# Atticuszz/GsplatLoc

Hardware: AMD Instinct MI355X
Metric: Gaussians/s fwd+bwd @1M splats 1200x680 (higher is better)
Workload: dtype f32

## Files before the change

### gsplatloc_amd/csrc/raster_g16.hip

```cpp
#include <stdlib.h>
#include <string.h>

#include "gsloc_common.h"

namespace gsl {

__device__ __forceinline__ float g16_sel(unsigned long long m, float t, float f) {
  float r;
  asm("v_cndmask_b32_e64 %0, %1, %2, %3" : "=v"(r) : "v"(f), "v"(t), "s"(m));
  return r;
}

#define G16_M_LO8 0x00FF00FF00FF00FFull
#define G16_M_B2 0x0F0F0F0F0F0F0F0Full
#define G16_M_B1 0x3333333333333333ull
#define G16_M_B0 0x5555555555555555ull

constexpr int G16_NG = GSL_NG;
constexpr int G16_GL = 64 / G16_NG;
static_assert(G16_NG == 4 || G16_NG == 8, "pixel groups are DPP rows or half rows");

__device__ __forceinline__ float row_scatter8(const float (&v)[8]) {
  float n0, n1, n2, n3, m0, m1;
  asm volatile(
      "s_nop 1\n\t"
      "v_add_f32_dpp %0, %6, %6 row_mirror row_mask:0xf bank_mask:0xf\n\t"
      "v_add_f32_dpp %1, %7, %7 row_mirror row_mask:0xf bank_mask:0xf\n\t"
      "v_add_f32_dpp %2, %8, %8 row_mirror row_mask:0xf bank_mask:0xf\n\t"
      "v_add_f32_dpp %3, %9, %9 row_mirror row_mask:0xf bank_mask:0xf\n\t"
      "v_add_f32_dpp %0, %10, %10 row_mirror row_mask:0xf bank_mask:0xc\n\t"
      "v_add_f32_dpp %1, %11, %11 row_mirror row_mask:0xf bank_mask:0xc\n\t"
      "v_add_f32_dpp %2, %12, %12 row_mirror row_mask:0xf bank_mask:0xc\n\t"
      "v_add_f32_dpp %4, %0, %0 row_half_mirror row_mask:0xf bank_mask:0xf\n\t"
      "v_add_f32_dpp %5, %1, %1 row_half_mirror row_mask:0xf bank_mask:0xf\n\t"
      "v_add_f32_dpp %4, %2, %2 row_half_mirror row_mask:0xf bank_mask:0xa\n\t"
      "v_add_f32_dpp %5, %3, %3 row_half_mirror row_mask:0xf bank_mask:0xa\n\t"
      : "=&v"(n0), "=&v"(n1), "=&v"(n2), "=&v"(n3), "=&v"(m0), "=&v"(m1)
      : "v"(v[0]), "v"(v[1]), "v"(v[2]), "v"(v[3]), "v"(v[4]), "v"(v[5]), "v"(v[6]));
  float keep = g16_sel(G16_M_B1, m0, m1), send = g16_sel(G16_M_B1, m1, m0);
  float r = keep + dpp_get<0x4E>(send);
  r += dpp_get<0xB1>(r);
  return r;
}

__device__ __forceinline__ float row_scatter16(const float (&v)[16]) {
  float a[8];
#pragma unroll
  for (int i = 0; i < 8; ++i) {
    float keep = g16_sel(G16_M_LO8, v[i], v[i + 8]), send = g16_sel(G16_M_LO8, v[i + 8], v[i]);
    a[i] = keep + dpp_get<0x140>(send);
  }
  float n[4], m[2];
#pragma unroll
  for (int i = 0; i < 4; ++i) {
    float keep = g16_sel(G16_M_B2, a[i], a[i + 4]), send = g16_sel(G16_M_B2, a[i + 4], a[i]);
    n[i] = keep + dpp_get<0x141>(send);
  }
#pragma unroll
  for (int i = 0; i < 2; ++i) {
    float keep = g16_sel(G16_M_B1, n[i], n[i + 2]), send = g16_sel(G16_M_B1, n[i + 2], n[i]);
    m[i] = keep + dpp_get<0x4E>(send);
  }
  float keep = g16_sel(G16_M_B0, m[0], m[1]), send = g16_sel(G16_M_B0, m[1], m[0]);
  return keep + dpp_get<0xB1>(send);
}

__device__ __forceinline__ float4 half_scatter8(const float (&v)[8]) {
  float n0, n1, n2, n3;
  asm volatile(
      "s_nop 1\n\t"
      "v_add_f32_dpp %0, %4, %4 row_half_mirror row_mask:0xf bank_mask:0xf\n\t"
      "v_add_f32_dpp %1, %5, %5 row_half_mirror row_mask:0xf bank_mask:0xf\n\t"
      "v_add_f32_dpp %2, %6, %6 row_half_mirror row_mask:0xf bank_mask:0xf\n\t"
      "v_add_f32_dpp %3, %7, %7 row_half_mirror row_mask:0xf bank_mask:0xf\n\t"
      "v_add_f32_dpp %0, %8, %8 row_half_mirror row_mask:0xf bank_mask:0xa\n\t"
      "v_add_f32_dpp %1, %9, %9 row_half_mirror row_mask:0xf bank_mask:0xa\n\t"
      "v_add_f32_dpp %2, %10, %10 row_half_mirror row_mask:0xf bank_mask:0xa\n\t"
      "s_nop 1\n\t"
      : "=&v"(n0), "=&v"(n1), "=&v"(n2), "=&v"(n3)
      : "v"(v[0]), "v"(v[1]), "v"(v[2]), "v"(v[3]), "v"(v[4]), "v"(v[5]), "v"(v[6]));
  n0 += dpp_get<0x4E>(n0); n1 += dpp_get<0x4E>(n1); n2 += dpp_get<0x4E>(n2); n3 += dpp_get<0x4E>(n3);
  n0 += dpp_get<0xB1>(n0); n1 += dpp_get<0xB1>(n1); n2 += dpp_get<0xB1>(n2); n3 += dpp_get<0xB1>(n3);
  return make_float4(n0, n1, n2, n3);
}

__device__ __forceinline__ void half_scatter16(const float (&v)[16], float4& lo, float4& hi) {
  float a[8];
#pragma unroll
  for (int i = 0; i < 8; ++i) {
    float keep = g16_sel(G16_M_B2, v[i], v[i + 8]), send = g16_sel(G16_M_B2, v[i + 8], v[i]);
    a[i] = keep + dpp_get<0x141>(send);
  }
#pragma unroll
  for (int i = 0; i < 8; ++i) a[i] += dpp_get<0x4E>(a[i]);
#pragma unroll
  for (int i = 0; i < 8; ++i) a[i] += dpp_get<0xB1>(a[i]);
  lo = make_float4(a[0], a[1], a[2], a[3]);
  hi = make_float4(a[4], a[5], a[6], a[7]);
}

#ifdef GSL_G16_STATS
__device__ unsigned long long g16_stats[8];
#define G16_STAT(i, n) do { unsigned long long n__ = (unsigned long long)(n); if (lane == 0) atomicAdd(&g16_stats[i], n__); } while (0)
#else
#define G16_STAT(i, n) do { } while (0)
#endif

#ifndef GSL_QB
#define GSL_QB 64
#endif
#define GSL_QBS (GSL_QB + 1)
#ifndef GSL_Q_LCAP
#define GSL_Q_LCAP 24
#endif

template <int D, int CG>
struct QStage {
  static constexpr int NV = 6 + CG;
  static constexpr int NS = (NV <= 8) ? 8 : 16;
  static constexpr int A = 6 + D;
  static constexpr int LCAP = ((NS == 8) ? GSL_Q_LCAP : GSL_Q_LCAP / 2) * 4 / G16_NG;
  float4 s0[GSL_QBS];
  float4 s1[GSL_QBS];
  float4 s2[(D >= 3 && CG == D) ? GSL_QBS : 1];
  int32_t id[GSL_QBS];
  uint32_t posn[G16_NG / 4][GSL_QBS];
  alignas(16) float pair[G16_NG * LCAP * NS];
  uint8_t rlist[G16_NG][GSL_QBS + 4];
  uint8_t nzlist[64];
};

template <int D, int CG>
__device__ __forceinline__ void qraster_bwd_body(
    QStage<D, CG>& sb, const float4* __restrict__ Q0, const float4* __restrict__ Q1, const float4* __restrict__ Q2,
    const uint4* __restrict__ Qh, const int32_t* __restrict__ flatten_ids, float* __restrict__ vacc, long long rs,
    long long re, int lane, int quad, float px, float py, float tx0, float ty0, int bin_final, float T_init,
    float Bp_init, const float (&vc)[D], const uint32_t* __restrict__ qhits, int n_qhits) {
  constexpr bool RGB = D >= 3;
  constexpr bool DEPTH = (D == 1) || (D == 4);
  constexpr int NV = QStage<D, CG>::NV;
  constexpr int NS = QStage<D, CG>::NS;
  constexpr int A = QStage<D, CG>::A;
  constexpr int LCAP = QStage<D, CG>::LCAP;
  constexpr int NG = G16_NG, GL = G16_GL;
  constexpr int PP = 12;
  static_assert(A <= PP && NG * LCAP * NS >= 64 * PP, "64 packed gradient rows reuse the pair slots");
  static_assert(GSL_QB < 127 && GSL_QB >= 64, "7-bit list positions with 127 reserved; a chunk appends up to 64 entries");
  const int grp = lane / GL, p = lane & (GL - 1);
  const float tcx = tx0 + 8.f, tcy = ty0 + 8.f;
  const float lx = px - tcx, ly = py - tcy;
  const float lxx = lx * lx, lxy = lx * ly, lyy = ly * ly;
  float T = T_init;
  float Bp = Bp_init;
  const int myslot = (NG == 8) ? (p >> 2) * (NS / 2) : ((NS == 8) ? (p >> 1) : p);
  const bool writer = (NG == 8) ? ((p & 3) == 0) : ((NS == 8) ? ((p & 1) == 0) : true);
  float* const mypair = &sb.pair[grp * LCAP * NS + myslot];
  uint8_t* const mylist = sb.rlist[grp];
  const unsigned long long lt = (1ull << lane) - 1ull;
  const float qx0 = tx0 + 8.f * (float)(quad & 1), qy0 = ty0 + 8.f * (float)(quad >> 1);
  int grp_final[NG];
  {
    int rf = bin_final;
    rf = max(rf, __shfl_xor(rf, 1, 64));
    rf = max(rf, __shfl_xor(rf, 2, 64));
    rf = max(rf, __shfl_xor(rf, 4, 64));
    if (GL == 16) rf = max(rf, __shfl_xor(rf, 8, 64));
#pragma unroll
    for (int g = 0; g < NG; ++g) grp_final[g] = __builtin_amdgcn_readlane(rf, GL * g);
  }
  if (lane == 0) {
    sb.s0[GSL_QB] = make_float4(0.f, 0.f, 0.f, 0.f);
    sb.s1[GSL_QB] = make_float4(0.f, 0.f, 0.f, 0.f);
    if (RGB && CG == D) sb.s2[GSL_QB] = make_float4(0.f, 0.f, 0.f, 0.f);
  }
  int pos = __builtin_amdgcn_readfirstlane(qhits ? n_qhits : (int)re);
  const int pos_end = __builtin_amdgcn_readfirstlane(qhits ? 0 : (int)rs);
  while (pos > pos_end) {
    int staged = 0;
    int cnt[NG];
#pragma unroll
    for (int g = 0; g < NG; ++g) cnt[g] = 0;
    __syncthreads();
    while (pos > pos_end && staged <= GSL_QB - 64) {
      long long idx = (long long)(pos - 1 - lane);
      bool in = idx >= (long long)pos_end;
      unsigned nib = 0;
      int gid = 0;
      float4 r0 = make_float4(0.f, 0.f, 0.f, 0.f), r1 = r0, r2 = r0;
      if (in) {
        if (qhits) {
          unsigned e = qhits[idx];
          nib = e >> GSL_HIT_SHIFT;
          idx = (long long)(e & GSL_HIT_INDEX_MASK);
          gid = flatten_ids[idx];
          load_record(Q0, Q1, Q2, Qh, gid, RGB && CG == D, r0, r1, r2);
        } else {
          gid = flatten_ids[idx];
          load_record(Q0, Q1, Q2, Qh, gid, RGB && CG == D, r0, r1, r2);
          if (r1.w >= 0.f) {
            float rr = r1.w * r1.w;
#pragma unroll
            for (int g = 0; g < NG; ++g) {
              const int b = (NG == 8) ? (g >> 1) : g;
              const float cy = (NG == 8) ? 2.f * (float)(g & 1) + 1.f : 2.f, hy = (NG == 8) ? 0.5f : 1.5f;
              float ex = fmaxf(fabsf(r0.x - (qx0 + 4.f * (float)(b & 1) + 2.f)) - 1.5f, 0.f);
              float ey = fmaxf(fabsf(r0.y - (qy0 + 4.f * (float)(b >> 1) + cy)) - hy, 0.f);
              bool h = (ex * ex + ey * ey <= rr) && ((int)idx <= grp_final[g]);
              nib |= (h ? 1u : 0u) << g;
            }
          }
        }
      }
      unsigned long long R = __ballot(nib != 0);
      int slot = staged + __popcll(R & lt);
      unsigned pack[NG / 4];
#pragma unroll
      for (int w = 0; w < NG / 4; ++w) pack[w] = 0x0FFFFFFFu;
#pragma unroll
      for (int g = 0; g < NG; ++g) {
        unsigned long long Bg = __ballot(nib & (1u << g));
        if (__builtin_amdgcn_inverse_ballot_w64(Bg)) {
          int q = cnt[g] + __popcll(Bg & lt);
          sb.rlist[g][q] = (uint8_t)slot;
          pack[g >> 2] ^= (127u ^ (unsigned)q) << (7 * (g & 3));
        }
        cnt[g] += __popcll(Bg);
      }
      if (__builtin_amdgcn_inverse_ballot_w64(R)) {
        sb.id[slot] = gid;
        sb.s0[slot] = r0;
        sb.s1[slot] = make_float4(r1.x * (0.5f * GSL_LOG2E), r1.y * GSL_LOG2E, r1.z * (0.5f * GSL_LOG2E),
                                  __int_as_float((int)idx));
        if (RGB && CG == D) sb.s2[slot] = r2;
#pragma unroll
        for (int w = 0; w < NG / 4; ++w) sb.posn[w][slot] = pack[w];
      }
      staged += __popcll(R);
      pos -= 64;
    }
    if (staged == 0) continue;
    int kmax = 0, cnt_tot = 0, cnt_my = 0;
#pragma unroll
    for (int g = 0; g < NG; ++g) {
      kmax = max(kmax, cnt[g]);
      cnt_tot += cnt[g];
      cnt_my = (grp == g) ? cnt[g] : cnt_my;
    }
    G16_STAT(6, kmax);
    G16_STAT(7, cnt_tot);
    (void)cnt_tot;
    for (int k = cnt_my + p; k < kmax + 3; k += GL) mylist[k] = (uint8_t)GSL_QB;
    __syncthreads();
    constexpr int NU = (GSL_QB + 63) / 64;
    float mo[NU][NV];
#pragma unroll
    for (int u = 0; u < NU; ++u)
#pragma unroll
      for (int q = 0; q < NV; ++q) mo[u][q] = 0.f;
    auto trip = [&](int t, const float4& c0, const float4& c1, float4& r, float4& r2) {
      float dx = c0.x - px, dy = c0.y - py;
      float sigma = fmaf(c1.y * dx, dy, fmaf(c1.x * dx, dx, c1.z * dy * dy));
      float vis = __builtin_amdgcn_exp2f(-sigma);
      float opv = c0.w * vis;
      float alpha = fminf(GSL_ALPHA_MAX, opv);
      unsigned long long validm = __ballot(__float_as_int(c1.w) <= bin_final) & __ballot(sigma >= 0.f) &
                                  __ballot(alpha >= GSL_ALPHA_MIN);
      G16_STAT(0, 1);
      r = make_float4(0.f, 0.f, 0.f, 0.f);
      r2 = r;
      if (validm) {
        G16_STAT(1, 1);
#ifdef GSL_G16_STATS
        {
          int groups_hit = 0;
          for (int g = 0; g < NG; ++g) groups_hit += ((validm >> (GL * g)) & ((1ull << GL) - 1ull)) != 0;
          G16_STAT(3, groups_hit);
        }
#endif
        G16_STAT(5, __popcll(validm));
        unsigned long long capm = __ballot(opv <= GSL_ALPHA_MAX);
        float am = g16_sel(validm, alpha, 0.f);
        float ra = __builtin_amdgcn_rcpf(1.f - am);
        T *= ra;
        float fac = am * T;
        float cdot;
        if (CG == D) {
          cdot = 0.f;
          if (RGB) {
            float4 q2 = sb.s2[t];
            cdot = q2.x * vc[0] + q2.y * vc[1] + q2.z * vc[2];
          }
          if (DEPTH) cdot += c0.z * vc[D - 1];
        } else {
          cdot = c0.z * vc[D - 1];
        }
        float v_alpha = T * cdot - ra * Bp;
        Bp += fac * cdot;
        float w = g16_sel(validm & capm, vis, 0.f) * v_alpha;
        float val[NS];
        val[0] = w; val[1] = w * lx; val[2] = w * ly; val[3] = w * lxx; val[4] = w * lxy; val[5] = w * lyy;
        if (CG == D) {
#pragma unroll
          for (int ch = 0; ch < D; ++ch) val[6 + ch] = fac * vc[ch];
        } else {
          val[6] = fac * vc[D - 1];
        }
#pragma unroll
        for (int q = NV; q < NS; ++q) val[q] = 0.f;
        static_assert(NS != 8 || NV == 7, "the 8-value scatters treat value 7 as padding");
        if (NG == 8) {
          if (NS == 8) r = half_scatter8(reinterpret_cast<const float(&)[8]>(val));
          else half_scatter16(reinterpret_cast<const float(&)[16]>(val), r, r2);
        } else {
          if (NS == 8) r.x = row_scatter8(reinterpret_cast<const float(&)[8]>(val));
          else r.x = row_scatter16(reinterpret_cast<const float(&)[16]>(val));
        }
      }
    };
    auto put = [&](float* dst, const float4& r, const float4& r2) {
      if (NG == 8) {
        *reinterpret_cast<float4*>(dst) = r;
        if (NS == 16) *reinterpret_cast<float4*>(dst + 4) = r2;
      } else {
        *dst = r.x;
      }
    };
    for (int k0 = 0; k0 < kmax; k0 += LCAP) {
      const int k1 = min(k0 + LCAP, kmax);
      int t0 = mylist[k0], t1 = mylist[k0 + 1];
      float4 qa0 = sb.s0[t0], qa1 = sb.s1[t0];
      float4 ra = make_float4(0.f, 0.f, 0.f, 0.f), ra2 = ra, rb = ra, rb2 = ra;
      float* dst = mypair;
      for (int k = k0; k < k1; k += 2) {
        if (k > k0 && writer) put(dst - NS, rb, rb2);
        const int t2 = mylist[k + 2];
        const float4 qb0 = sb.s0[t1], qb1 = sb.s1[t1];
        trip(t0, qa0, qa1, ra, ra2);
        if (writer) put(dst, ra, ra2);
        const int t3 = mylist[k + 3];
        qa0 = sb.s0[t2];
        qa1 = sb.s1[t2];
        trip(t1, qb0, qb1, rb, rb2);
        t0 = t2;
        t1 = t3;
        dst += 2 * NS;
      }
      if (writer) put(dst - NS, rb, rb2);
      __syncthreads();
#pragma unroll
      for (int u = 0; u < NU; ++u) {
        int slot = lane + 64 * u;
        if (slot < staged) {
#pragma unroll
          for (int w = 0; w < NG / 4; ++w) {
            unsigned pk = sb.posn[w][slot];
#pragma unroll
            for (int g4 = 0; g4 < 4; ++g4) {
              const int g = 4 * w + g4;
              const unsigned q = ((pk >> (7 * g4)) & 127u) - (unsigned)k0;
              if (q < (unsigned)LCAP) {
                const float4* src = reinterpret_cast<const float4*>(&sb.pair[(g * LCAP + q) * NS]);
                float4 a = src[0], c = src[1];
                mo[u][0] += a.x; mo[u][1] += a.y; mo[u][2] += a.z; mo[u][3] += a.w;
                mo[u][4] += c.x; mo[u][5] += c.y; mo[u][6] += c.z;
                if (NV > 7) mo[u][7 < NV ? 7 : 0] += c.w;
                if (NS == 16) {
                  float4 e = src[2];
                  if (NV > 8) mo[u][8 < NV ? 8 : 0] += e.x;
                  if (NV > 9) mo[u][9 < NV ? 9 : 0] += e.y;
                }
              }
            }
          }
        }
      }
      __syncthreads();
    }
#pragma unroll
    for (int u = 0; u < NU; ++u) {
      int slot = lane + 64 * u;
      bool nz = false;
      float row[A];
#pragma unroll
      for (int k = 0; k < A; ++k) row[k] = 0.f;
      if (slot < staged) {
        {
          unsigned bits = 0u;
#pragma unroll
          for (int k = 0; k < NV; ++k) bits |= __float_as_uint(mo[u][k]);
          nz = (bits << 1) != 0u;
        }
        if (nz) {
          float4 r0 = sb.s0[slot], r1 = sb.s1[slot];
          float X = r0.x - tcx, Y = r0.y - tcy, S = mo[u][0];
          float Sx = X * S - mo[u][1], Sy = Y * S - mo[u][2];
          float Sxx = X * (X * S - 2.f * mo[u][1]) + mo[u][3];
          float Sxy = X * (Y * S - mo[u][2]) - Y * mo[u][1] + mo[u][4];
          float Syy = Y * (Y * S - 2.f * mo[u][2]) + mo[u][5];
          float no = -r0.w;
          r1.x *= 2.f / GSL_LOG2E; r1.y *= 1.f / GSL_LOG2E; r1.z *= 2.f / GSL_LOG2E;
          row[0] = no * (r1.x * Sx + r1.y * Sy);
          row[1] = no * (r1.y * Sx + r1.z * Sy);
          row[2] = 0.5f * no * Sxx;
          row[3] = no * Sxy;
          row[4] = 0.5f * no * Syy;
          row[5] = S;
          if (CG == D) {
#pragma unroll
            for (int ch = 0; ch < D; ++ch) row[6 + ch] = mo[u][6 + ch];
          } else {
            row[6 + D - 1] = mo[u][6];
          }
        }
      }
      float* packed = sb.pair;
      if (nz) {
#pragma unroll
        for (int k = 0; k < A; ++k) packed[lane * PP + k] = row[k];
      }
      unsigned long long mask = __ballot(nz);
      int cntz = __popcll(mask);
      if (nz) sb.nzlist[__popcll(mask & lt)] = (uint8_t)lane;
      __syncthreads();
      constexpr int RPI = 64 / A;
      const int arow = lane / A, f = lane - arow * A;
      for (int i0 = 0; i0 < cntz; i0 += RPI) {
        int gi = i0 + arow;
        if (gi < cntz && arow < RPI) {
          int sl = sb.nzlist[gi];
          const unsigned off = ((unsigned)sb.id[sl + 64 * u] << 6) | ((unsigned)f << 2);
          atomicAdd(reinterpret_cast<float*>(reinterpret_cast<char*>(vacc) + off), packed[sl * PP + f]);
        }
      }
      __syncthreads();
    }
  }
}

template <int D, bool ED, int CG, bool LONG>
__device__ __forceinline__ void qraster_bwd_item(
    QStage<D, CG>& sb, int b, int n_items, const float4* __restrict__ Q0, const float4* __restrict__ Q1,
    const float4* __restrict__ Q2, int W, int H, int tile_w, int ty0, const int32_t* __restrict__ tile_offsets,
    const int32_t* __restrict__ flatten_ids, long long capacity, const float* __restrict__ render,
    const float* __restrict__ alphas, const int32_t* __restrict__ last_ids, const float* __restrict__ v_render,
    const float* __restrict__ v_alphas, float* __restrict__ vacc, int row0, int row1, const uint4* __restrict__ Qh,
    const uint32_t* __restrict__ isect_hits, int32_t* __restrict__ isect_hit_counts, int long_min, LongWs lw,
    int32_t* __restrict__ rgb_flag, int32_t* __restrict__ clear_counts, int32_t* __restrict__ clear_state) {
  if (!LONG && (CG == 1 || D == 3) && clear_counts && (b & 3) == 0 && threadIdx.x == 0) {
    clear_counts[ty0 * tile_w + (b >> 2)] = 0;
    if (b == 0 && clear_state) *clear_state = 0;
  }
  const int wi = LONG ? b : xcd_span_item(b, n_items);
  const int quad = wi & 3, item = wi >> 2;
  int tile, sgm = 0, gseg = 0;
  if (LONG) {
    gseg = item;
    if (gseg >= lw.n_seg[0]) return;
    tile = lw.seg_tile[gseg];
    sgm = lw.seg_idx[gseg];
    if (tile < 0) return;
  } else {
    tile = ty0 * tile_w + item;
  }
  int tyi = tile / tile_w, txi = tile - tyi * tile_w;
  int lane = threadIdx.x, grp = lane >> 4, p = lane & 15;
  int j = txi * 16 + (quad & 1) * 8 + (grp & 1) * 4 + (p & 3);
  int i = tyi * 16 + (quad >> 1) * 8 + (grp >> 1) * 4 + (p >> 2);
  float px = (float)j + 0.5f, py = (float)i + 0.5f;
  bool inside = (i < H) && (j < W) && (i >= row0) && (i < row1);

  long long rs = tile_offsets[tile], re = tile_offsets[tile + 1];
  if (re > capacity) re = capacity;
  if (rs >= re) return;
  if (!LONG && long_min > 0 && re - rs > long_min) return;
  if (LONG) {
    rs += (long long)sgm * GSL_SEG;
    re = min(rs + (long long)GSL_SEG, re);
  }
  size_t pid = inside ? ((size_t)i * W + j) : 0;
  int bin_final = inside ? last_ids[pid] : -1;
  int quad_final = bin_final;
#pragma unroll
  for (int o = 32; o >= 1; o >>= 1) quad_final = max(quad_final, __shfl_xor(quad_final, o, 64));
  if ((long long)quad_final + 1 < re) re = (long long)quad_final + 1;
  if (rs >= re) return;
  float vc[D];
#pragma unroll
  for (int k = 0; k < D; ++k) vc[k] = inside ? v_render[pid * D + k] : 0.f;
  if (D == 4) {
    bool rgb_grad = (vc[0] != 0.f) || (vc[1] != 0.f) || (vc[2] != 0.f);
    bool any_rgb = __ballot(rgb_grad) != 0ull;
    if ((CG == 1) == any_rgb) {
      if (CG == 1 && rgb_flag && lane == 0) atomicOr(rgb_flag, 1);
      return;
    }
  }
  float Aimg = inside ? alphas[pid] : 0.f;
  float T_final = 1.f - Aimg;
  float va = inside ? v_alphas[pid] : 0.f;
  if (ED && inside) {
    float dn = render[pid * D + (D - 1)];
    float vd = vc[D - 1];
    if (Aimg >= 1e-10f) va += -vd * dn / Aimg;
    vc[D - 1] = vd / fmaxf(Aimg, 1e-10f);
  }
  float T_init = T_final, Bp_init = -T_final * va;
  if (LONG) {
    int nseg = lw.seg_cnt[gseg];
    long long seg_end = min(tile_offsets[tile] + (long long)(sgm + 1) * GSL_SEG, (long long)tile_offsets[tile + 1]);
    int pslot = quad * 64 + lane;
    if (inside && (long long)bin_final >= seg_end) {
      T_init = fabsf(lw.Tend[(size_t)gseg * 256 + pslot]);
      const float4* C4 = reinterpret_cast<const float4*>(lw.C);
      bool stop = false;
      for (int s0 = sgm + 1; s0 < nseg && !stop; s0 += 8) {
        float t8[8];
        float4 c8[8];
#pragma unroll
        for (int u = 0; u < 8; ++u) {
          size_t slot = (size_t)(gseg - sgm + min(s0 + u, nseg - 1)) * 256 + pslot;
          t8[u] = lw.Tend[slot];
          c8[u] = C4[slot];
        }
#pragma unroll
        for (int u = 0; u < 8; ++u) {
          if (stop || s0 + u >= nseg) continue;
          if (t8[u] == 2.f) { stop = true; continue; }
          float cc[4] = {c8[u].x, c8[u].y, c8[u].z, c8[u].w};
          float dot = 0.f;
#pragma unroll
          for (int k = 0; k < D; ++k) dot += vc[k] * cc[k];
          Bp_init += dot;
          if (t8[u] < 0.f) stop = true;
        }
      }
    }
  }
  const uint32_t* qh = nullptr;
  int nqh = 0;
  if (isect_hits) {
    long long ls = tile_offsets[tile], le = tile_offsets[tile + 1];
    if (le > capacity) le = capacity;
    if (LONG) {
      ls += (long long)sgm * GSL_SEG;
      le = min(ls + (long long)GSL_SEG, le);
      nqh = lw.seg_qcnt[gseg * 4 + quad];
    } else {
      nqh = isect_hit_counts[tile * 4 + quad];
    }
    qh = isect_hits + 4 * ls + (long long)quad * (le - ls);
    if (nqh == 0) return;
  }
  qraster_bwd_body<D, CG>(sb, Q0, Q1, Q2, Qh, flatten_ids, vacc, rs, re, lane, quad, px, py, (float)(txi * 16),
                          (float)(tyi * 16), bin_final, T_init, Bp_init, vc, qh, nqh);
}

template <int D, bool ED, int CG, bool LONG>
__global__ __launch_bounds__(64) void k_qraster_bwd(
    const float4* __restrict__ Q0, const float4* __restrict__ Q1, const float4* __restrict__ Q2, int W, int H,
    int tile_w, int ty0, const int32_t* __restrict__ tile_offsets, const int32_t* __restrict__ flatten_ids,
    long long capacity, const float* __restrict__ render, const float* __restrict__ alphas,
    const int32_t* __restrict__ last_ids, const float* __restrict__ v_render, const float* __restrict__ v_alphas,
    float* __restrict__ vacc, int row0, int row1, const uint4* __restrict__ Qh,
    const uint32_t* __restrict__ isect_hits, int32_t* __restrict__ isect_hit_counts, int long_min, LongWs lw,
    int32_t* __restrict__ rgb_flag, int32_t* __restrict__ clear_counts, int32_t* __restrict__ clear_state, int n_items) {
  __shared__ QStage<D, CG> sb;
  if (D == 4 && CG == D && rgb_flag && *rgb_flag == 0) return;
  for (int b = (int)blockIdx.x; b < n_items; b += (int)gridDim.x) {
    qraster_bwd_item<D, ED, CG, LONG>(sb, b, n_items, Q0, Q1, Q2, W, H, tile_w, ty0, tile_offsets, flatten_ids, capacity,
                                      render, alphas, last_ids, v_render, v_alphas, vacc, row0, row1, Qh, isect_hits,
                                      isect_hit_counts, long_min, lw, rgb_flag, clear_counts, clear_state);
    __syncthreads();
  }
}

}

#ifdef GSL_G16_STATS
extern "C" int gsl_g16_stats(unsigned long long* host_out, int reset) {
  if (hipMemcpyFromSymbol(host_out, HIP_SYMBOL(gsl::g16_stats), sizeof(unsigned long long) * 8) != hipSuccess) return -3;
  if (reset) {
    unsigned long long z[8] = {0};
    if (hipMemcpyToSymbol(HIP_SYMBOL(gsl::g16_stats), z, sizeof(z)) != hipSuccess) return -3;
  }
  return 0;
}
#endif

extern "C" int32_t* gsl_fused_bin_state(void* ws, int n_tiles);

extern "C" int gsl_g16_raster_bwd_launch(const float* Q0, const float* Q1, const float* Q2, int channels, int ed, int width,
                                         int height, int tile_w, int ty0, int ty1, const int32_t* tile_offsets,
                                         const int32_t* flatten_ids, int64_t capacity, const float* render,
                                         const float* alphas, const int32_t* last_ids, const float* v_render,
                                         const float* v_alphas, float* vacc, int row0, int row1, const void* Qh,
                                         const uint32_t* isect_hits, const int32_t* isect_hit_counts, int long_min,
                                         void* long_ws, int max_seg, int rgb_flag_index, void* clear_ws,
                                         void* stream) {
  hipStream_t st = (hipStream_t)stream;
  int nblk = long_ws ? max_seg : (ty1 - ty0) * tile_w;
  gsl::LongWs lw = gsl::long_ws_views(long_ws ? long_ws : (void*)0, long_ws ? max_seg : 0);
  const bool lng = long_ws != nullptr;
  int32_t* rgb_flag = isect_hit_counts ? const_cast<int32_t*>(isect_hit_counts) + rgb_flag_index : nullptr;
  int32_t* clear_counts = (int32_t*)clear_ws;
  int32_t* clear_state = clear_ws ? gsl_fused_bin_state(clear_ws, rgb_flag_index / 4) : nullptr;
#define CALL_Q(DD, EE, CC)                                                                                   \
  do {                                                                                                       \
    const int n_items = 4 * nblk;                                                                            \
    const int grid = ((DD) == 4 && (CC) == 4 && rgb_flag && n_items > 2048) ? 2048 : n_items;                \
    if (lng)                                                                                                 \
      hipLaunchKernelGGL((gsl::k_qraster_bwd<DD, EE, CC, true>), dim3(grid), dim3(64), 0, st, (const float4*)Q0, \
                         (const float4*)Q1, (const float4*)Q2, width, height, tile_w, ty0, tile_offsets,     \
                         flatten_ids, (long long)capacity, render, alphas, last_ids, v_render, v_alphas, vacc, \
                         row0, row1, (const uint4*)Qh, isect_hits, const_cast<int32_t*>(isect_hit_counts), long_min, lw, rgb_flag, clear_counts, clear_state, n_items);                   \
    else                                                                                                     \
      hipLaunchKernelGGL((gsl::k_qraster_bwd<DD, EE, CC, false>), dim3(grid), dim3(64), 0, st, (const float4*)Q0, \
                         (const float4*)Q1, (const float4*)Q2, width, height, tile_w, ty0, tile_offsets,     \
                         flatten_ids, (long long)capacity, render, alphas, last_ids, v_render, v_alphas, vacc, \
                         row0, row1, (const uint4*)Qh, isect_hits, const_cast<int32_t*>(isect_hit_counts), long_min, lw, rgb_flag, clear_counts, clear_state, n_items);                   \
  } while (0)
  if (channels == 1) { if (ed) CALL_Q(1, true, 1); else CALL_Q(1, false, 1); }
  else if (channels == 3) { CALL_Q(3, false, 3); }
  else if (channels == 4) {
    if (ed) { CALL_Q(4, true, 1); CALL_Q(4, true, 4); }
    else { CALL_Q(4, false, 1); CALL_Q(4, false, 4); }
  }
  else return GSL_ERR_BAD_ARG;
#undef CALL_Q
  GSL_CHECK_LAUNCH();
  return GSL_OK;
}
```

Baseline: 2.428 billion.

## Specialize backward raster on hit-list mode and streamline staging and gradient scatter

Templates the backward raster body on whether precomputed hit lists exist, giving two kernels and letting the compiler drop the unused path. Staging now uses mbcnt ranks, scalar max and popcount, and clears the per-group lists with dword stores instead of per-group byte loops. The gradient scatter packs nonzero rows compactly with the pre-shifted gaussian offset stored in the row, removing the nzlist indirection and the separate id lookup during atomics. This trims per-chunk instruction overhead and LDS traffic, at the cost of more code variants and tighter static assumptions on row width.

```diff
diff --git a/gsplatloc_amd/csrc/raster_g16.hip b/gsplatloc_amd/csrc/raster_g16.hip
--- a/gsplatloc_amd/csrc/raster_g16.hip
+++ b/gsplatloc_amd/csrc/raster_g16.hip
@@ -10,6 +10,26 @@
   asm("v_cndmask_b32_e64 %0, %1, %2, %3" : "=v"(r) : "v"(f), "v"(t), "s"(m));
   return r;
 }
+
+__device__ __forceinline__ unsigned g16_sel_u32(unsigned long long m, unsigned t, unsigned f) {
+  unsigned r;
+  asm("v_cndmask_b32_e64 %0, %1, %2, %3" : "=v"(r) : "v"(f), "v"(t), "s"(m));
+  return r;
+}
+__device__ __forceinline__ int g16_rank(unsigned long long m, int base) {
+  return (int)__builtin_amdgcn_mbcnt_hi((unsigned)(m >> 32), __builtin_amdgcn_mbcnt_lo((unsigned)m, (unsigned)base));
+}
+__device__ __forceinline__ int g16_smax(int a, int b) {
+  int r;
+  asm("s_max_i32 %0, %1, %2" : "=s"(r) : "s"(a), "s"(b) : "scc");
+  return r;
+}
+__device__ __forceinline__ int g16_popc(unsigned long long m) {
+  int r;
+  asm("s_bcnt1_i32_b64 %0, %1" : "=s"(r) : "s"(m) : "scc");
+  return r;
+}
+__device__ __forceinline__ unsigned long long g16_first_lanes(int n) { return n >= 64 ? ~0ull : (1ull << n) - 1ull; }
 
 #define G16_M_LO8 0x00FF00FF00FF00FFull
 #define G16_M_B2 0x0F0F0F0F0F0F0F0Full
@@ -123,14 +143,14 @@
   float4 s0[GSL_QBS];
   float4 s1[GSL_QBS];
   float4 s2[(D >= 3 && CG == D) ? GSL_QBS : 1];
-  int32_t id[GSL_QBS];
+  uint32_t idoff[GSL_QBS];
   uint32_t posn[G16_NG / 4][GSL_QBS];
   alignas(16) float pair[G16_NG * LCAP * NS];
-  uint8_t rlist[G16_NG][GSL_QBS + 4];
-  uint8_t nzlist[64];
+  alignas(4) uint8_t rlist[G16_NG][GSL_QBS + 4];
+  static_assert((G16_NG * (GSL_QBS + 4)) % 4 == 0, "the lists are cleared as dwords");
 };
 
-template <int D, int CG>
+template <int D, int CG, bool HL>
 __device__ __forceinline__ void qraster_bwd_body(
     QStage<D, CG>& sb, const float4* __restrict__ Q0, const float4* __restrict__ Q1, const float4* __restrict__ Q2,
     const uint4* __restrict__ Qh, const int32_t* __restrict__ flatten_ids, float* __restrict__ vacc, long long rs,
@@ -144,7 +164,7 @@
   constexpr int LCAP = QStage<D, CG>::LCAP;
   constexpr int NG = G16_NG, GL = G16_GL;
   constexpr int PP = 12;
-  static_assert(A <= PP && NG * LCAP * NS >= 64 * PP, "64 packed gradient rows reuse the pair slots");
+  static_assert(A < PP && NG * LCAP * NS >= 64 * PP, "64 packed gradient rows reuse the pair slots");
   static_assert(GSL_QB < 127 && GSL_QB >= 64, "7-bit list positions with 127 reserved; a chunk appends up to 64 entries");
   const int grp = lane / GL, p = lane & (GL - 1);
   const float tcx = tx0 + 8.f, tcy = ty0 + 8.f;
@@ -156,10 +176,9 @@
   const bool writer = (NG == 8) ? ((p & 3) == 0) : ((NS == 8) ? ((p & 1) == 0) : true);
   float* const mypair = &sb.pair[grp * LCAP * NS + myslot];
   uint8_t* const mylist = sb.rlist[grp];
-  const unsigned long long lt = (1ull << lane) - 1ull;
   const float qx0 = tx0 + 8.f * (float)(quad & 1), qy0 = ty0 + 8.f * (float)(quad >> 1);
   int grp_final[NG];
-  {
+  if constexpr (!HL) {
     int rf = bin_final;
     rf = max(rf, __shfl_xor(rf, 1, 64));
     rf = max(rf, __shfl_xor(rf, 2, 64));
@@ -168,69 +187,82 @@
 #pragma unroll
     for (int g = 0; g < NG; ++g) grp_final[g] = __builtin_amdgcn_readlane(rf, GL * g);
   }
+  (void)qx0; (void)qy0; (void)grp_final;
   if (lane == 0) {
     sb.s0[GSL_QB] = make_float4(0.f, 0.f, 0.f, 0.f);
     sb.s1[GSL_QB] = make_float4(0.f, 0.f, 0.f, 0.f);
     if (RGB && CG == D) sb.s2[GSL_QB] = make_float4(0.f, 0.f, 0.f, 0.f);
   }
-  int pos = __builtin_amdgcn_readfirstlane(qhits ? n_qhits : (int)re);
-  const int pos_end = __builtin_amdgcn_readfirstlane(qhits ? 0 : (int)rs);
+  int pos = __builtin_amdgcn_readfirstlane(HL ? n_qhits : (int)re);
+  const int pos_end = HL ? 0 : __builtin_amdgcn_readfirstlane((int)rs);
   while (pos > pos_end) {
     int staged = 0;
     int cnt[NG];
 #pragma unroll
     for (int g = 0; g < NG; ++g) cnt[g] = 0;
     __syncthreads();
+    {
+      constexpr int NW = NG * (GSL_QBS + 4) / 4;
+      uint32_t* const words = reinterpret_cast<uint32_t*>(&sb.rlist[0][0]);
+#pragma unroll
+      for (int w0 = 0; w0 < NW; w0 += 64) {
+        if (NW - w0 >= 64) {
+          words[w0 + lane] = 0x01010101u * (unsigned)GSL_QB;
+        } else if (__builtin_amdgcn_inverse_ballot_w64((1ull << ((NW - w0) & 63)) - 1ull)) {
+          words[w0 + lane] = 0x01010101u * (unsigned)GSL_QB;
+        }
+      }
+    }
     while (pos > pos_end && staged <= GSL_QB - 64) {
-      long long idx = (long long)(pos - 1 - lane);
-      bool in = idx >= (long long)pos_end;
-      unsigned nib = 0;
-      int gid = 0;
-      float4 r0 = make_float4(0.f, 0.f, 0.f, 0.f), r1 = r0, r2 = r0;
-      if (in) {
-        if (qhits) {
-          unsigned e = qhits[idx];
-          nib = e >> GSL_HIT_SHIFT;
-          idx = (long long)(e & GSL_HIT_INDEX_MASK);
-          gid = flatten_ids[idx];
-          load_record(Q0, Q1, Q2, Qh, gid, RGB && CG == D, r0, r1, r2);
-        } else {
-          gid = flatten_ids[idx];
-          load_record(Q0, Q1, Q2, Qh, gid, RGB && CG == D, r0, r1, r2);
-          if (r1.w >= 0.f) {
-            float rr = r1.w * r1.w;
-#pragma unroll
-            for (int g = 0; g < NG; ++g) {
-              const int b = (NG == 8) ? (g >> 1) : g;
-              const float cy = (NG == 8) ? 2.f * (float)(g & 1) + 1.f : 2.f, hy = (NG == 8) ? 0.5f : 1.5f;
-              float ex = fmaxf(fabsf(r0.x - (qx0 + 4.f * (float)(b & 1) + 2.f)) - 1.5f, 0.f);
-              float ey = fmaxf(fabsf(r0.y - (qy0 + 4.f * (float)(b >> 1) + cy)) - hy, 0.f);
-              bool h = (ex * ex + ey * ey <= rr) && ((int)idx <= grp_final[g]);
-              nib |= (h ? 1u : 0u) << g;
-            }
+      const unsigned long long IN = g16_first_lanes(pos - pos_end);
+      int idx = max(pos - 1 - lane, pos_end);
+      unsigned hits = 0;
+      int gid;
+      float4 r0, r1, r2 = make_float4(0.f, 0.f, 0.f, 0.f);
+      if constexpr (HL) {
+        hits = qhits[idx];
+        idx = (int)(hits & GSL_HIT_INDEX_MASK);
+        gid = flatten_ids[idx];
+        load_record(Q0, Q1, Q2, Qh, gid, RGB && CG == D, r0, r1, r2);
+      } else {
+        gid = flatten_ids[idx];
+        load_record(Q0, Q1, Q2, Qh, gid, RGB && CG == D, r0, r1, r2);
+        if (r1.w >= 0.f) {
+          float rr = r1.w * r1.w;
+#pragma unroll
+          for (int g = 0; g < NG; ++g) {
+            const int b = (NG == 8) ? (g >> 1) : g;
+            const float cy = (NG == 8) ? 2.f * (float)(g & 1) + 1.f : 2.f, hy = (NG == 8) ? 0.5f : 1.5f;
+            float ex = fmaxf(fabsf(r0.x - (qx0 + 4.f * (float)(b & 1) + 2.f)) - 1.5f, 0.f);
+            float ey = fmaxf(fabsf(r0.y - (qy0 + 4.f * (float)(b >> 1) + cy)) - hy, 0.f);
+            bool h = (ex * ex + ey * ey <= rr) && (idx <= grp_final[g]);
+            hits |= (h ? 1u : 0u) << (GSL_HIT_SHIFT + g);
           }
         }
       }
-      unsigned long long R = __ballot(nib != 0);
-      int slot = staged + __popcll(R & lt);
+      unsigned long long Bg[NG], R = 0ull;
+#pragma unroll
+      for (int g = 0; g < NG; ++g) {
+        Bg[g] = IN & __ballot((hits & (1u << (GSL_HIT_SHIFT + g))) != 0u);
+        R |= Bg[g];
+      }
+      constexpr bool ONE = GSL_QB == 64;
+      const int slot = g16_rank(R, ONE ? 0 : staged);
       unsigned pack[NG / 4];
 #pragma unroll
-      for (int w = 0; w < NG / 4; ++w) pack[w] = 0x0FFFFFFFu;
+      for (int w = 0; w < NG / 4; ++w) pack[w] = 0u;
 #pragma unroll
       for (int g = 0; g < NG; ++g) {
-        unsigned long long Bg = __ballot(nib & (1u << g));
-        if (__builtin_amdgcn_inverse_ballot_w64(Bg)) {
-          int q = cnt[g] + __popcll(Bg & lt);
-          sb.rlist[g][q] = (uint8_t)slot;
-          pack[g >> 2] ^= (127u ^ (unsigned)q) << (7 * (g & 3));
-        }
-        cnt[g] += __popcll(Bg);
+        const int q = g16_rank(Bg[g], ONE ? 0 : cnt[g]);
+        if (__builtin_amdgcn_inverse_ballot_w64(Bg[g])) sb.rlist[g][q] = (uint8_t)slot;
+        pack[g >> 2] |= g16_sel_u32(Bg[g], (unsigned)q, 127u) << (7 * (g & 3));
+        cnt[g] += __popcll(Bg[g]);
       }
       if (__builtin_amdgcn_inverse_ballot_w64(R)) {
-        sb.id[slot] = gid;
+        sb.idoff[slot] = (unsigned)gid << 6;
         sb.s0[slot] = r0;
         sb.s1[slot] = make_float4(r1.x * (0.5f * GSL_LOG2E), r1.y * GSL_LOG2E, r1.z * (0.5f * GSL_LOG2E),
-                                  __int_as_float((int)idx));
+                                  __int_as_float(idx));
         if (RGB && CG == D) sb.s2[slot] = r2;
 #pragma unroll
         for (int w = 0; w < NG / 4; ++w) sb.posn[w][slot] = pack[w];
@@ -239,17 +271,15 @@
       pos -= 64;
     }
     if (staged == 0) continue;
-    int kmax = 0, cnt_tot = 0, cnt_my = 0;
-#pragma unroll
-    for (int g = 0; g < NG; ++g) {
-      kmax = max(kmax, cnt[g]);
+    int kmax = cnt[0], cnt_tot = cnt[0];
+#pragma unroll
+    for (int g = 1; g < NG; ++g) {
+      kmax = g16_smax(kmax, cnt[g]);
       cnt_tot += cnt[g];
-      cnt_my = (grp == g) ? cnt[g] : cnt_my;
     }
     G16_STAT(6, kmax);
     G16_STAT(7, cnt_tot);
     (void)cnt_tot;
-    for (int k = cnt_my + p; k < kmax + 3; k += GL) mylist[k] = (uint8_t)GSL_QB;
     __syncthreads();
     constexpr int NU = (GSL_QB + 63) / 64;
     float mo[NU][NV];
@@ -378,66 +408,60 @@
     }
 #pragma unroll
     for (int u = 0; u < NU; ++u) {
-      int slot = lane + 64 * u;
-      bool nz = false;
-      float row[A];
-#pragma unroll
-      for (int k = 0; k < A; ++k) row[k] = 0.f;
-      if (slot < staged) {
-        {
-          unsigned bits = 0u;
-#pragma unroll
-          for (int k = 0; k < NV; ++k) bits |= __float_as_uint(mo[u][k]);
-          nz = (bits << 1) != 0u;
-        }
-        if (nz) {
-          float4 r0 = sb.s0[slot], r1 = sb.s1[slot];
-          float X = r0.x - tcx, Y = r0.y - tcy, S = mo[u][0];
-          float Sx = X * S - mo[u][1], Sy = Y * S - mo[u][2];
-          float Sxx = X * (X * S - 2.f * mo[u][1]) + mo[u][3];
-          float Sxy = X * (Y * S - mo[u][2]) - Y * mo[u][1] + mo[u][4];
-          float Syy = Y * (Y * S - 2.f * mo[u][2]) + mo[u][5];
-          float no = -r0.w;
-          r1.x *= 2.f / GSL_LOG2E; r1.y *= 1.f / GSL_LOG2E; r1.z *= 2.f / GSL_LOG2E;
-          row[0] = no * (r1.x * Sx + r1.y * Sy);
-          row[1] = no * (r1.y * Sx + r1.z * Sy);
-          row[2] = 0.5f * no * Sxx;
-          row[3] = no * Sxy;
-          row[4] = 0.5f * no * Syy;
-          row[5] = S;
-          if (CG == D) {
-#pragma unroll
-            for (int ch = 0; ch < D; ++ch) row[6 + ch] = mo[u][6 + ch];
-          } else {
-            row[6 + D - 1] = mo[u][6];
+      const int slot = lane + 64 * u;
+      unsigned bits = 0u;
+#pragma unroll
+      for (int k = 0; k < NV; ++k) bits |= __float_as_uint(mo[u][k]);
+      const unsigned long long NZ = __ballot((bits << 1) != 0u);
+      const int cntz = g16_popc(NZ);
+      constexpr int AL = (CG == D) ? A : 7;
+      constexpr int IDW = (AL < 8) ? 7 : PP - 1;
+      float* packed = sb.pair;
+      if (__builtin_amdgcn_inverse_ballot_w64(NZ)) {
+        float row[PP];
+#pragma unroll
+        for (int k = 0; k < PP; ++k) row[k] = 0.f;
+        float4 r0 = sb.s0[slot], r1 = sb.s1[slot];
+        float X = r0.x - tcx, Y = r0.y - tcy, S = mo[u][0];
+        float Sx = X * S - mo[u][1], Sy = Y * S - mo[u][2];
+        float Sxx = X * (X * S - 2.f * mo[u][1]) + mo[u][3];
+        float Sxy = X * (Y * S - mo[u][2]) - Y * mo[u][1] + mo[u][4];
+        float Syy = Y * (Y * S - 2.f * mo[u][2]) + mo[u][5];
+        float no = -r0.w;
+        r1.x *= 2.f / GSL_LOG2E; r1.y *= 1.f / GSL_LOG2E; r1.z *= 2.f / GSL_LOG2E;
+        row[0] = no * (r1.x * Sx + r1.y * Sy);
+        row[1] = no * (r1.y * Sx + r1.z * Sy);
+        row[2] = 0.5f * no * Sxx;
+        row[3] = no * Sxy;
+        row[4] = 0.5f * no * Syy;
+        row[5] = S;
+#pragma unroll
+        for (int k = 6; k < AL; ++k) row[k] = mo[u][k];
+        row[IDW] = __uint_as_float(sb.idoff[slot]);
+        float4* dst = reinterpret_cast<float4*>(&packed[g16_rank(NZ, 0) * PP]);
+#pragma unroll
+        for (int k = 0; k <= IDW / 4; ++k) dst[k] = make_float4(row[4 * k], row[4 * k + 1], row[4 * k + 2], row[4 * k + 3]);
+      }
+      __syncthreads();
+      constexpr int RPI = 64 / AL;
+      const int arow = lane / AL, fl = lane - arow * AL;
+      const int f = (CG == D || fl < 6) ? fl : 6 + D - 1;
+      const float* const src = packed + arow * PP;
+#pragma unroll
+      for (int i0 = 0; i0 < 64; i0 += RPI) {
+        if (i0 < cntz) {
+          if (__builtin_amdgcn_inverse_ballot_w64(g16_first_lanes(min(cntz - i0, RPI) * AL))) {
+            const unsigned off = __float_as_uint(src[i0 * PP + IDW]) | ((unsigned)f << 2);
+            atomicAdd(reinterpret_cast<float*>(reinterpret_cast<char*>(vacc) + off), src[i0 * PP + fl]);
           }
         }
       }
-      float* packed = sb.pair;
-      if (nz) {
-#pragma unroll
-        for (int k = 0; k < A; ++k) packed[lane * PP + k] = row[k];
-      }
-      unsigned long long mask = __ballot(nz);
-      int cntz = __popcll(mask);
-      if (nz) sb.nzlist[__popcll(mask & lt)] = (uint8_t)lane;
       __syncthreads();
-      constexpr int RPI = 64 / A;
-      const int arow = lane / A, f = lane - arow * A;
-      for (int i0 = 0; i0 < cntz; i0 += RPI) {
-        int gi = i0 + arow;
-        if (gi < cntz && arow < RPI) {
-          int sl = sb.nzlist[gi];
-          const unsigned off = ((unsigned)sb.id[sl + 64 * u] << 6) | ((unsigned)f << 2);
-          atomicAdd(reinterpret_cast<float*>(reinterpret_cast<char*>(vacc) + off), packed[sl * PP + f]);
-        }
-      }
-      __syncthreads();
-    }
-  }
-}
-
-template <int D, bool ED, int CG, bool LONG>
+    }
+  }
+}
+
+template <int D, bool ED, int CG, bool LONG, bool HL>
 __device__ __forceinline__ void qraster_bwd_item(
     QStage<D, CG>& sb, int b, int n_items, const float4* __restrict__ Q0, const float4* __restrict__ Q1,
     const float4* __restrict__ Q2, int W, int H, int tile_w, int ty0, const int32_t* __restrict__ tile_offsets,
@@ -538,7 +562,7 @@
   }
   const uint32_t* qh = nullptr;
   int nqh = 0;
-  if (isect_hits) {
+  if constexpr (HL) {
     long long ls = tile_offsets[tile], le = tile_offsets[tile + 1];
     if (le > capacity) le = capacity;
     if (LONG) {
@@ -551,28 +575,43 @@
     qh = isect_hits + 4 * ls + (long long)quad * (le - ls);
     if (nqh == 0) return;
   }
-  qraster_bwd_body<D, CG>(sb, Q0, Q1, Q2, Qh, flatten_ids, vacc, rs, re, lane, quad, px, py, (float)(txi * 16),
+  qraster_bwd_body<D, CG, HL>(sb, Q0, Q1, Q2, Qh, flatten_ids, vacc, rs, re, lane, quad, px, py, (float)(txi * 16),
                           (float)(tyi * 16), bin_final, T_init, Bp_init, vc, qh, nqh);
 }
 
-template <int D, bool ED, int CG, bool LONG>
-__global__ __launch_bounds__(64) void k_qraster_bwd(
-    const float4* __restrict__ Q0, const float4* __restrict__ Q1, const float4* __restrict__ Q2, int W, int H,
-    int tile_w, int ty0, const int32_t* __restrict__ tile_offsets, const int32_t* __restrict__ flatten_ids,
-    long long capacity, const float* __restrict__ render, const float* __restrict__ alphas,
-    const int32_t* __restrict__ last_ids, const float* __restrict__ v_render, const float* __restrict__ v_alphas,
-    float* __restrict__ vacc, int row0, int row1, const uint4* __restrict__ Qh,
-    const uint32_t* __restrict__ isect_hits, int32_t* __restrict__ isect_hit_counts, int long_min, LongWs lw,
-    int32_t* __restrict__ rgb_flag, int32_t* __restrict__ clear_counts, int32_t* __restrict__ clear_state, int n_items) {
-  __shared__ QStage<D, CG> sb;
+#define GSL_QRASTER_BWD_PARAMS                                                                                        \
+  const float4 *__restrict__ Q0, const float4 *__restrict__ Q1, const float4 *__restrict__ Q2, int W, int H, int tile_w, \
+      int ty0, const int32_t *__restrict__ tile_offsets, const int32_t *__restrict__ flatten_ids, long long capacity,    \
+      const float *__restrict__ render, const float *__restrict__ alphas, const int32_t *__restrict__ last_ids,          \
+      const float *__restrict__ v_render, const float *__restrict__ v_alphas, float *__restrict__ vacc, int row0,        \
+      int row1, const uint4 *__restrict__ Qh, const uint32_t *__restrict__ isect_hits,                                   \
+      int32_t *__restrict__ isect_hit_counts, int long_min, LongWs lw, int32_t *__restrict__ rgb_flag,                   \
+      int32_t *__restrict__ clear_counts, int32_t *__restrict__ clear_state, int n_items
+template <int D, bool ED, int CG, bool LONG, bool HL>
+__device__ __forceinline__ void qraster_bwd_kernel(QStage<D, CG>& sb, GSL_QRASTER_BWD_PARAMS) {
   if (D == 4 && CG == D && rgb_flag && *rgb_flag == 0) return;
   for (int b = (int)blockIdx.x; b < n_items; b += (int)gridDim.x) {
-    qraster_bwd_item<D, ED, CG, LONG>(sb, b, n_items, Q0, Q1, Q2, W, H, tile_w, ty0, tile_offsets, flatten_ids, capacity,
-                                      render, alphas, last_ids, v_render, v_alphas, vacc, row0, row1, Qh, isect_hits,
-                                      isect_hit_counts, long_min, lw, rgb_flag, clear_counts, clear_state);
+    qraster_bwd_item<D, ED, CG, LONG, HL>(sb, b, n_items, Q0, Q1, Q2, W, H, tile_w, ty0, tile_offsets, flatten_ids,
+                                          capacity, render, alphas, last_ids, v_render, v_alphas, vacc, row0, row1, Qh,
+                                          isect_hits, isect_hit_counts, long_min, lw, rgb_flag, clear_counts, clear_state);
     __syncthreads();
   }
 }
+#define GSL_QRASTER_BWD_ARGS                                                                                           \
+  Q0, Q1, Q2, W, H, tile_w, ty0, tile_offsets, flatten_ids, capacity, render, alphas, last_ids, v_render, v_alphas, vacc, \
+      row0, row1, Qh, isect_hits, isect_hit_counts, long_min, lw, rgb_flag, clear_counts, clear_state, n_items
+template <int D, bool ED, int CG, bool LONG>
+__global__ __launch_bounds__(64) void k_qraster_bwd(GSL_QRASTER_BWD_PARAMS) {
+  __shared__ QStage<D, CG> sb;
+  qraster_bwd_kernel<D, ED, CG, LONG, true>(sb, GSL_QRASTER_BWD_ARGS);
+}
+template <int D, bool ED, int CG, bool LONG>
+__global__ __launch_bounds__(64) void k_qraster_bwd_nohits(GSL_QRASTER_BWD_PARAMS) {
+  __shared__ QStage<D, CG> sb;
+  qraster_bwd_kernel<D, ED, CG, LONG, false>(sb, GSL_QRASTER_BWD_ARGS);
+}
+#undef GSL_QRASTER_BWD_ARGS
+#undef GSL_QRASTER_BWD_PARAMS
 
 }
 
@@ -604,20 +643,22 @@
   int32_t* rgb_flag = isect_hit_counts ? const_cast<int32_t*>(isect_hit_counts) + rgb_flag_index : nullptr;
   int32_t* clear_counts = (int32_t*)clear_ws;
   int32_t* clear_state = clear_ws ? gsl_fused_bin_state(clear_ws, rgb_flag_index / 4) : nullptr;
-#define CALL_Q(DD, EE, CC)                                                                                   \
-  do {                                                                                                       \
-    const int n_items = 4 * nblk;                                                                            \
-    const int grid = ((DD) == 4 && (CC) == 4 && rgb_flag && n_items > 2048) ? 2048 : n_items;                \
-    if (lng)                                                                                                 \
-      hipLaunchKernelGGL((gsl::k_qraster_bwd<DD, EE, CC, true>), dim3(grid), dim3(64), 0, st, (const float4*)Q0, \
-                         (const float4*)Q1, (const float4*)Q2, width, height, tile_w, ty0, tile_offsets,     \
-                         flatten_ids, (long long)capacity, render, alphas, last_ids, v_render, v_alphas, vacc, \
-                         row0, row1, (const uint4*)Qh, isect_hits, const_cast<int32_t*>(isect_hit_counts), long_min, lw, rgb_flag, clear_counts, clear_state, n_items);                   \
-    else                                                                                                     \
-      hipLaunchKernelGGL((gsl::k_qraster_bwd<DD, EE, CC, false>), dim3(grid), dim3(64), 0, st, (const float4*)Q0, \
-                         (const float4*)Q1, (const float4*)Q2, width, height, tile_w, ty0, tile_offsets,     \
-                         flatten_ids, (long long)capacity, render, alphas, last_ids, v_render, v_alphas, vacc, \
-                         row0, row1, (const uint4*)Qh, isect_hits, const_cast<int32_t*>(isect_hit_counts), long_min, lw, rgb_flag, clear_counts, clear_state, n_items);                   \
+#define CALL_QK(KERNEL, DD, EE, CC, LL)                                                                               \
+  hipLaunchKernelGGL((gsl::KERNEL<DD, EE, CC, LL>), dim3(grid), dim3(64), 0, st, (const float4*)Q0, (const float4*)Q1,  \
+                     (const float4*)Q2, width, height, tile_w, ty0, tile_offsets, flatten_ids, (long long)capacity,     \
+                     render, alphas, last_ids, v_render, v_alphas, vacc, row0, row1, (const uint4*)Qh, isect_hits,      \
+                     const_cast<int32_t*>(isect_hit_counts), long_min, lw, rgb_flag, clear_counts, clear_state, n_items)
+#define CALL_Q(DD, EE, CC)                                                                    \
+  do {                                                                                        \
+    const int n_items = 4 * nblk;                                                             \
+    const int grid = ((DD) == 4 && (CC) == 4 && rgb_flag && n_items > 2048) ? 2048 : n_items; \
+    if (isect_hits) {                                                                         \
+      if (lng) CALL_QK(k_qraster_bwd, DD, EE, CC, true);                                      \
+      else CALL_QK(k_qraster_bwd, DD, EE, CC, false);                                         \
+    } else {                                                                                  \
+      if (lng) CALL_QK(k_qraster_bwd_nohits, DD, EE, CC, true);                               \
+      else CALL_QK(k_qraster_bwd_nohits, DD, EE, CC, false);                                  \
+    }                                                                                         \
   } while (0)
   if (channels == 1) { if (ed) CALL_Q(1, true, 1); else CALL_Q(1, false, 1); }
   else if (channels == 3) { CALL_Q(3, false, 3); }
@@ -627,6 +668,7 @@
   }
   else return GSL_ERR_BAD_ARG;
 #undef CALL_Q
+#undef CALL_QK
   GSL_CHECK_LAUNCH();
   return GSL_OK;
 }
```

After: 2.450 billion, median of 6. About the same (+0.9%).
